# KadAMRN/Data_Free_Quantization

Hardware: AMD Instinct MI355X
Metric: weight-GB/s quantized (per-ch INT8 DFQ sweep) + top-1 delta, MobileNetV2 (higher is better)
Workload: dtype f32

## Files before the change

data_free_quantization_amd/csrc/dfq_sweep.hip:

```cpp
#include "dfq_common.h"
#include "dfq_sweep_plan.h"
#ifdef DFQ_DIAGNOSTICS
#include "dfq_diag.h"
#endif

#include <algorithm>
#include <cstring>
#include <cstdlib>
#include <new>
#include <type_traits>
#include <vector>

namespace dfq {

constexpr int kBlockThreads = kWave * kWavesPerBlock;

__device__ __forceinline__ int64_t task_elem_start(const DevTask& k, const DevTensor& T) { return k.src - T.src; }

template <int CHUNK, int MAXROWS, int NB>
struct LdsLayout {
    static constexpr int kPerWave = NB * CHUNK + 3 * MAXROWS;
    static constexpr int kTotal = kWavesPerBlock * kPerWave;
};

__device__ __forceinline__ bool is_sym(int mode) { return mode == DFQ_TENSOR_SYM || mode == DFQ_CHANNEL_SYM; }

template <bool NT, typename V>
__device__ __forceinline__ void st(V* p, const V& v);

__device__ __forceinline__ void store_code(void* codes, int cb, int64_t idx, float q) {
    if (cb == 1) {
        st<false>(static_cast<int8_t*>(codes) + idx, (int8_t)(int)q);
    } else {
        st<false>(static_cast<int16_t*>(codes) + idx, (int16_t)(int)q);
    }
}

typedef __attribute__((address_space(3))) void lds_void_t;
typedef __attribute__((address_space(1))) void gbl_void_t;

template <bool NT = false>
__device__ __forceinline__ void glds16(const float* g, float* lds_base) {
    __builtin_amdgcn_global_load_lds((gbl_void_t*)g, (lds_void_t*)lds_base, 16, 0, NT ? 2 : 0);
}
template <bool NT = false>
__device__ __forceinline__ void glds4(const float* g, float* lds_base) {
    __builtin_amdgcn_global_load_lds((gbl_void_t*)g, (lds_void_t*)lds_base, 4, 0, NT ? 2 : 0);
}
template <bool NT = false>
__device__ __forceinline__ void glds16_asm(const float* g, float* lds_base) {
    const uint32_t m0 = (uint32_t)(uintptr_t)(lds_void_t*)lds_base;
    if constexpr (NT) asm volatile("global_load_lds_dwordx4 %0, off nt" ::"v"(g), "{m0}"(m0) : "memory");
    else asm volatile("global_load_lds_dwordx4 %0, off" ::"v"(g), "{m0}"(m0) : "memory");
}
template <bool NT = false>
__device__ __forceinline__ void glds4_asm(const float* g, float* lds_base) {
    const uint32_t m0 = (uint32_t)(uintptr_t)(lds_void_t*)lds_base;
    if constexpr (NT) asm volatile("global_load_lds_dword %0, off nt" ::"v"(g), "{m0}"(m0) : "memory");
    else asm volatile("global_load_lds_dword %0, off" ::"v"(g), "{m0}"(m0) : "memory");
}
typedef float f32x4 __attribute__((ext_vector_type(4)));
template <bool NT, typename V>
__device__ __forceinline__ void st(V* p, const V& v) {
    if constexpr (sizeof(V) == 16) {
        const f32x4 w = {v.x, v.y, v.z, v.w};
        DFQ_GLOBAL f32x4* g = (DFQ_GLOBAL f32x4*)p;
        if constexpr (NT) __builtin_nontemporal_store(w, g);
        else *g = w;
    } else {
        DFQ_GLOBAL V* g = (DFQ_GLOBAL V*)p;
        if constexpr (NT) __builtin_nontemporal_store(v, g);
        else *g = v;
    }
}
__device__ __forceinline__ float ld(const float* p) { return *(const DFQ_GLOBAL float*)p; }
__device__ __forceinline__ float4 ld(const float4* p) {
    const f32x4 v = *(const DFQ_GLOBAL f32x4*)p;
    return make_float4(v.x, v.y, v.z, v.w);
}
__device__ __forceinline__ void vm_wait_all() { asm volatile("s_waitcnt vmcnt(0)" ::: "memory"); }

__global__ void __launch_bounds__(kBlockThreads)
sweep_reduce_kernel(const DevTensor* __restrict__ tensors, const DevTask* __restrict__ tasks,
                    int64_t ntasks, uint32_t* __restrict__ slot_min, uint32_t* __restrict__ slot_max) {
    const int lane = threadIdx.x & (kWave - 1);
    const int64_t wave0 = (int64_t)blockIdx.x * kWavesPerBlock + wave_uniform(threadIdx.x >> 6);
    const int64_t nwaves = (int64_t)gridDim.x * kWavesPerBlock;
    for (int64_t t = wave0; t < ntasks; t += nwaves) {
        const DevTask task = tasks[t];
        const float* src = task.src;
        float vmin = INFINITY, vmax = -INFINITY;
        if (task.flags & 2) {
            const int nj = task.n >> 2;
#pragma unroll 8
            for (int j = lane; j < nj; j += kWave) {
                const float4 v = ld(reinterpret_cast<const float4*>(src) + j);
                vmin = fminf(vmin, fminf(fminf(v.x, v.y), fminf(v.z, v.w)));
                vmax = fmaxf(vmax, fmaxf(fmaxf(v.x, v.y), fmaxf(v.z, v.w)));
            }
        } else {
#pragma unroll 8
            for (int e = lane; e < task.n; e += kWave) {
                const float x = ld(src + e);
                vmin = fminf(vmin, x);
                vmax = fmaxf(vmax, x);
            }
        }
        vmin = wave_min(vmin);
        vmax = wave_max(vmax);
        if (lane == 0) {
            atomicMin(&slot_min[task.slot], enc_ord(vmin));
            atomicMax(&slot_max[task.slot], enc_ord(vmax));
        }
    }
}

template <bool NT = false, bool ASM = false>
__device__ __forceinline__ void issue_task_load(const DevTask& task, float* data, int lane) {
    const float* src = task.src;
    const int n = task.n;
    if (task.flags & 2) {
        const int nj = n >> 2;
        for (int m = 0; m * kWave < nj; ++m) {
            const int j = lane + m * kWave;
            if (j < nj) {
                if constexpr (ASM) glds16_asm<NT>(src + 4 * j, data + 4 * kWave * m);
                else glds16<NT>(src + 4 * j, data + 4 * kWave * m);
            }
        }
    } else {
        for (int m = 0; m * kWave < n; ++m) {
            const int e = lane + m * kWave;
            if (e < n) {
                if constexpr (ASM) glds4_asm<NT>(src + e, data + kWave * m);
                else glds4<NT>(src + e, data + kWave * m);
            }
        }
    }
}


typedef float f32x2 __attribute__((ext_vector_type(2)));
template <bool CLIP, int CB, int EM, bool NT>
__device__ __forceinline__ void quant_vec4(const DevTensor& T, int n, int64_t base, float* data, const float* ls,
                                           const float* lmn, const float* lrs, const QParams& pc, bool whole,
                                           int eoff, int lane, float qmin, float qmax, bool sym) {
    constexpr float kMagic = 12582912.0f;
    const int nj = n >> 2;
    float* dq = T.dst + base;
    const float clo = T.clip_lo, chi = T.clip_hi;
    const uint32_t magic = whole ? T.len_magic : 0u;
    const float thr = 0.5f - fmaxf(-qmin, qmax) * 0x1p-20f;
    const f32x2 mg = {kMagic, kMagic};
    struct Q4 {
        float4 x;
        float s, mn;
        float t[4];
        f32x2 ta, tb, qa, qb, da, db;
    };
    auto prep = [&](int j, uint32_t e, Q4& q) {
        q.x = reinterpret_cast<const float4*>(data)[j];
        const uint32_t r = __umulhi(e, magic);
        q.s = ls[r];
        q.mn = lmn[r];
        const float rs = lrs[r];
        const f32x2 nm = {-q.mn, -q.mn};
        const f32x2 rs2 = {rs, rs};
        const f32x2 a = (f32x2{q.x.x, q.x.y} + nm) * rs2, b = (f32x2{q.x.z, q.x.w} + nm) * rs2;
        q.t[0] = __builtin_amdgcn_fmed3f(a.x, qmin, qmax);
        q.t[1] = __builtin_amdgcn_fmed3f(a.y, qmin, qmax);
        q.t[2] = __builtin_amdgcn_fmed3f(b.x, qmin, qmax);
        q.t[3] = __builtin_amdgcn_fmed3f(b.y, qmin, qmax);
        q.ta = f32x2{q.t[0], q.t[1]} + mg;
        q.tb = f32x2{q.t[2], q.t[3]} + mg;
        q.qa = q.ta - mg;
        q.qb = q.tb - mg;
        asm("" : "+v"(q.ta), "+v"(q.tb), "+v"(q.qa), "+v"(q.qb));
        q.da = f32x2{q.t[0], q.t[1]} - q.qa;
        q.db = f32x2{q.t[2], q.t[3]} - q.qb;
    };
    auto dmax = [&](const Q4& q) { return fmaxf(fmaxf(fabsf(q.da.x), fabsf(q.da.y)), fmaxf(fabsf(q.db.x), fabsf(q.db.y))); };
    auto fix = [&](Q4& q) {
        const float negmn = -q.mn;
        if (fabsf(q.da.x) >= thr) q.t[0] = __builtin_amdgcn_fmed3f((q.x.x + negmn) / q.s, qmin, qmax);
        if (fabsf(q.da.y) >= thr) q.t[1] = __builtin_amdgcn_fmed3f((q.x.y + negmn) / q.s, qmin, qmax);
        if (fabsf(q.db.x) >= thr) q.t[2] = __builtin_amdgcn_fmed3f((q.x.z + negmn) / q.s, qmin, qmax);
        if (fabsf(q.db.y) >= thr) q.t[3] = __builtin_amdgcn_fmed3f((q.x.w + negmn) / q.s, qmin, qmax);
        q.ta = f32x2{q.t[0], q.t[1]} + mg;
        q.tb = f32x2{q.t[2], q.t[3]} + mg;
        q.qa = q.ta - mg;
        q.qb = q.tb - mg;
    };
    auto out = [&](int j, const Q4& q) {
        const f32x2 s2 = {q.s, q.s}, mn2 = {q.mn, q.mn};
        const f32x2 ya = q.qa * s2 + mn2, yb = q.qb * s2 + mn2;
        float y[4] = {ya.x, ya.y, yb.x, yb.y};
        if constexpr (CLIP) {
#pragma unroll
            for (int k = 0; k < 4; ++k) y[k] = __builtin_amdgcn_fmed3f(y[k], clo, chi);
        }
        st<NT>(reinterpret_cast<float4*>(dq) + j, make_float4(y[0], y[1], y[2], y[3]));
        const uint32_t u0 = __float_as_uint(q.ta.x), u1 = __float_as_uint(q.ta.y);
        const uint32_t u2 = __float_as_uint(q.tb.x), u3 = __float_as_uint(q.tb.y);
        if constexpr (CB == 1) {
            const uint32_t c = __builtin_amdgcn_perm(u1, u0, 0x0c0c0400u) | __builtin_amdgcn_perm(u3, u2, 0x04000c0cu);
            st<NT>(reinterpret_cast<uint32_t*>(static_cast<uint8_t*>(T.codes) + base) + j, c);
        } else if constexpr (CB == 3) {
            const uint32_t c = (u0 & 0xFu) | ((u1 & 0xFu) << 4) | ((u2 & 0xFu) << 8) | ((u3 & 0xFu) << 12);
            st<NT>(reinterpret_cast<uint16_t*>(static_cast<uint8_t*>(T.codes) + base / 2) + j, (uint16_t)c);
        } else if constexpr (CB == 2) {
            const uint64_t c = (uint64_t)__builtin_amdgcn_perm(u1, u0, 0x05040100u) |
                               ((uint64_t)__builtin_amdgcn_perm(u3, u2, 0x05040100u) << 32);
            st<NT>(reinterpret_cast<uint64_t*>(static_cast<uint16_t*>(T.codes) + base) + j, c);
        }
        if constexpr (EM != 0) {
            const f32x2 ea = f32x2{y[0], y[1]} - f32x2{q.x.x, q.x.y}, eb = f32x2{y[2], y[3]} - f32x2{q.x.z, q.x.w};
            const float4 ev = make_float4(ea.x, ea.y, eb.x, eb.y);
            if constexpr (EM == 1) st<NT>(reinterpret_cast<float4*>(T.esum + base) + j, ev);
            else reinterpret_cast<float4*>(data)[j] = ev;
        }
    };
    uint32_t e = (uint32_t)(4 * lane + eoff);
    for (int j = lane; j < nj; j += 2 * kWave, e += 8 * kWave) {
        const int j1 = j + kWave;
        const bool has1 = j1 < nj;
        Q4 qa, qb;
        prep(j, e, qa);
        prep(has1 ? j1 : j, has1 ? e + 4 * kWave : e, qb);
        if (__builtin_amdgcn_ballot_w64(fmaxf(dmax(qa), dmax(qb)) >= thr)) {
            fix(qa);
            fix(qb);
        }
        out(j, qa);
        if (has1) out(j1, qb);
    }
}

template <bool CLIP, int CB, bool NT>
__device__ __forceinline__ void quant_vec4_e(int em, const DevTensor& T, int n, int64_t base, float* data,
                                             const float* ls, const float* lmn, const float* lrs, const QParams& pc,
                                             bool whole, int eoff, int lane, float qmin, float qmax, bool sym) {
    if (em == 0) quant_vec4<CLIP, CB, 0, NT>(T, n, base, data, ls, lmn, lrs, pc, whole, eoff, lane, qmin, qmax, sym);
    else if (em == 1) quant_vec4<CLIP, CB, 1, NT>(T, n, base, data, ls, lmn, lrs, pc, whole, eoff, lane, qmin, qmax, sym);
    else quant_vec4<CLIP, CB, 2, NT>(T, n, base, data, ls, lmn, lrs, pc, whole, eoff, lane, qmin, qmax, sym);
}

template <bool CLIP, bool NT>
__device__ __forceinline__ void quant_vec4_c(int cb, int em, const DevTensor& T, int n, int64_t base, float* data,
                                             const float* ls, const float* lmn, const float* lrs, const QParams& pc,
                                             bool whole, int eoff, int lane, float qmin, float qmax, bool sym) {
    switch (cb) {
        case 0: quant_vec4_e<CLIP, 0, NT>(em, T, n, base, data, ls, lmn, lrs, pc, whole, eoff, lane, qmin, qmax, sym); break;
        case 1: quant_vec4_e<CLIP, 1, NT>(em, T, n, base, data, ls, lmn, lrs, pc, whole, eoff, lane, qmin, qmax, sym); break;
        case 2: quant_vec4_e<CLIP, 2, NT>(em, T, n, base, data, ls, lmn, lrs, pc, whole, eoff, lane, qmin, qmax, sym); break;
        default: quant_vec4_e<CLIP, 3, NT>(em, T, n, base, data, ls, lmn, lrs, pc, whole, eoff, lane, qmin, qmax, sym);
    }
}

template <int MAXROWS, bool VEC, bool NT = false, int ESPEC = 2, bool SCREEN = true, bool FAST = true>
__device__ __forceinline__ void compute_task(const DevTensor& T, const DevTask& task, float* data, float* ls,
                                             float* lmn, const uint32_t* __restrict__ slot_min,
                                             const uint32_t* __restrict__ slot_max, int lane, float bmn = 0.f,
                                             float bmx = 0.f, int goff = -1, uint64_t* tlm = nullptr,
                                             uint32_t abl = 0) {
    const int n = task.n;
    const bool sym = is_sym(T.mode);
// ... 488 lines not shown
                        gmn = fminf(gmn, b0[q * P + MAXROWS + rr]);
                    }
                }
                block_lds_sync();
                if (rr <= rl) {
                    const QParams p = make_qparams(gmn, gmx, T.bits, is_sym(T.mode), T.flags, T.given_min,
                                                   T.given_max);
                    ls[lane] = p.s;
                    lmn[lane] = p.mn;
                    lmn[MAXROWS + lane] = __builtin_amdgcn_rcpf(p.s);
                    if (rr * len >= g0) {
                        const int64_t row_g = task.row0 + rr;
                        if (T.scale) st<false>(T.scale + row_g, p.s);
                        if (T.zero) st<false>(T.zero + row_g, p.mn);
                    }
                }
                wave_lds_sync();
                goff = g0 - rf * len;
            } else if (task.nrows < 0) {
                float vmin = INFINITY, vmax = -INFINITY;
                if (T.vec4) {
                    for (int j = lane; j < (task.n >> 2); j += kWave) {
                        const float4 v = reinterpret_cast<const float4*>(wl)[j];
                        vmin = fminf(vmin, fminf(fminf(v.x, v.y), fminf(v.z, v.w)));
                        vmax = fmaxf(vmax, fmaxf(fmaxf(v.x, v.y), fmaxf(v.z, v.w)));
                    }
                } else {
                    for (int e = lane; e < task.n; e += kWave) {
                        vmin = fminf(vmin, wl[e]);
                        vmax = fmaxf(vmax, wl[e]);
                    }
                }
                vmin = wave_min(vmin);
                vmax = wave_max(vmax);
                if (lane == 0) {
                    ls[0] = vmin;
                    ls[1] = vmax;
                }
                block_lds_sync();
                constexpr int P = Lay::kPerWave;
                if (task.nrows == -kWavesPerBlock) {
                    const float* b0 = lds + NB * CHUNK;
                    bmn = fminf(fminf(b0[0], b0[P]), fminf(b0[2 * P], b0[3 * P]));
                    bmx = fmaxf(fmaxf(b0[1], b0[P + 1]), fmaxf(b0[2 * P + 1], b0[3 * P + 1]));
                } else {
                    const float* b0 = lds + (w & ~1) * P + NB * CHUNK;
                    bmn = fminf(b0[0], b0[P]);
                    bmx = fmaxf(b0[1], b0[P + 1]);
                }
                block_lds_sync();
            }
            uint64_t marks[4] = {0, 0, 0, 0};
            uint64_t* tlm = TL ? marks : nullptr;
            if (T.vec4)
                compute_task<MAXROWS, true, NT, ESPEC, SCREEN, FAST>(T, task, wl, ls, lmn, slot_min, slot_max, lane,
                                                                     bmn, bmx, goff, tlm, abl);
            else
                compute_task<MAXROWS, false, NT, ESPEC, SCREEN, FAST>(T, task, wl, ls, lmn, slot_min, slot_max, lane,
                                                                      bmn, bmx, goff, tlm, abl);
            if constexpr (TL) {
                if (lane == 0 && t < g_timeline_cap) {
                    uint32_t hw;
                    asm volatile("s_getreg_b32 %0, hwreg(HW_REG_HW_ID)" : "=s"(hw));
                    uint32_t xcc;
                    asm volatile("s_getreg_b32 %0, hwreg(HW_REG_XCC_ID)" : "=s"(xcc));
                    const uint64_t tl2 = wall_clock64();
                    uint64_t* r = g_timeline + 8 * t;
                    r[0] = tl0;
                    r[1] = tl1;
                    r[2] = marks[0];
                    r[3] = marks[1];
                    r[4] = tl2;
                    r[5] = ((uint64_t)task.tensor << 40) | ((uint64_t)(xcc & 0xFF) << 32) | hw;
                    r[6] = marks[2];
                    r[7] = marks[3];
                }
            }
            task = next;
        }
    } else {
        int cur = 0;
        int64_t t = wave0;
        if (t < ntasks) {
            const DevTask task = tasks[t];
            issue_task_load<NT>(task, wl, lane);
        }
        for (; t < ntasks; t += nwaves) {
            const DevTask task = tasks[t];
            const DevTensor T = tensors[task.tensor];
            vm_wait_all();
            wave_lds_sync();
            const int64_t tn = t + nwaves;
            if (tn < ntasks) {
                const DevTask nt = tasks[tn];
                issue_task_load<NT>(nt, wl + (cur ^ 1) * CHUNK, lane);
            }
            float* data = wl + cur * CHUNK;
            if (T.vec4) compute_task<MAXROWS, true, NT, ESPEC, SCREEN>(T, task, data, ls, lmn, slot_min, slot_max, lane);
            else compute_task<MAXROWS, false, NT, ESPEC, SCREEN>(T, task, data, ls, lmn, slot_min, slot_max, lane);
            cur ^= 1;
        }
    }
}

static int lds_bytes(const Variant& V) {
    return 4 * kWavesPerBlock * ((V.prefetch ? 2 : 1) * V.chunk + 3 * V.max_rows);
}

using MainKernel = void (*)(const DevTensor*, const DevTask*, int64_t, const uint32_t*, const uint32_t*);

static MainKernel main_kernel(int variant) {
#define DFQ_V(i) kVariants[i].chunk, kVariants[i].max_rows, kVariants[i].prefetch
#ifndef DFQ_DIAGNOSTICS
    if (variant == kSmallVariant) return sweep_main_kernel<DFQ_V(kSmallVariant), true, 1>;
    return sweep_main_kernel<DFQ_V(kDefaultVariant), true, 1, false, true, true, kDefaultVariant == 16>;
#else
    switch (variant) {
        case 1: return sweep_main_kernel<DFQ_V(1)>;
        case 2: return sweep_main_kernel<DFQ_V(2)>;
        case 3: return sweep_main_kernel<DFQ_V(3)>;
        case 4: return sweep_main_kernel<DFQ_V(4)>;
        case 5: return sweep_main_kernel<DFQ_V(5), true>;
        case 6: return sweep_main_kernel<DFQ_V(6), true, 1>;
        case 7: return sweep_main_kernel<DFQ_V(7), true, 0>;
        case 8: return sweep_main_kernel<DFQ_V(8), true, 1>;
        case 9: return sweep_main_kernel<DFQ_V(9), true, 1>;
        case 10: return sweep_main_kernel<DFQ_V(10), true, 1>;
        case 11: return sweep_main_kernel<DFQ_V(11), true, 1>;
        case 12: return sweep_main_kernel<DFQ_V(12), true, 0>;
        case 13: return sweep_main_kernel<DFQ_V(13), true, 1, true>;
        case 14: return sweep_main_kernel<DFQ_V(14), true, 1, false, false>;
        case 15: return sweep_main_kernel<DFQ_V(15), true, 1, false, true, false>;
        case 16: return sweep_main_kernel<DFQ_V(16), true, 1, false, true, true, true>;
        default: return sweep_main_kernel<DFQ_V(0)>;
    }
#endif
#undef DFQ_V
}

constexpr int kBlocksPerCu = 64;
static int blocks_per_cu() {
    static const int v = [] {
        const char* e = ab_env("DFQ_SWEEP_BLOCKS_PER_CU");
        return e && *e ? std::max(1, std::min(1024, atoi(e))) : kBlocksPerCu;
    }();
    return v;
}
static int grid_for(int64_t ntasks) {
    const int64_t want = ceil_div(ntasks, kWavesPerBlock);
    return (int)std::max<int64_t>(1, std::min<int64_t>(want, 256 * (int64_t)blocks_per_cu()));
}

static int launch_sweep(int variant, hipStream_t s, const DevTensor* t, const DevTask* reduce, int64_t n_reduce,
                        const DevTask* main, int64_t n_main, uint32_t* slots, int64_t n_slots) {
    if (n_reduce > 0) {
        DFQ_HIP_CHECK(hipMemsetAsync(slots, 0xFF, sizeof(uint32_t) * n_slots, s));
        DFQ_HIP_CHECK(hipMemsetAsync(slots + n_slots, 0x00, sizeof(uint32_t) * n_slots, s));
        hipLaunchKernelGGL(sweep_reduce_kernel, dim3(grid_for(n_reduce)), dim3(kBlockThreads), 0, s, t, reduce,
                           n_reduce, slots, slots + n_slots);
        DFQ_LAUNCH_CHECK();
    }
    if (n_main > 0) {
        hipLaunchKernelGGL(main_kernel(variant), dim3(grid_for(n_main)), dim3(kBlockThreads), 0, s, t, main, n_main,
                           slots, slots + n_slots);
        DFQ_LAUNCH_CHECK();
    }
    return DFQ_OK;
}

static std::vector<char> table_blob(const SweepTables& T, size_t o_tensors, size_t o_reduce, size_t o_main,
                                    size_t end) {
    std::vector<char> blob(end - o_tensors, 0);
    auto put = [&](size_t off, const void* p, size_t bytes) {
        if (bytes) std::memcpy(blob.data() + (off - o_tensors), p, bytes);
    };
    put(o_tensors, T.tensors.data(), sizeof(DevTensor) * T.tensors.size());
    put(o_reduce, T.reduce.data(), sizeof(DevTask) * T.reduce.size());
    put(o_main, T.main.data(), sizeof(DevTask) * T.main.size());
    return blob;
}

}

using namespace dfq;

struct dfq_sweep_plan {
    int variant = kDefaultVariant;
    DevTensor* d_tensors = nullptr;
    DevTask* d_reduce = nullptr;
    DevTask* d_main = nullptr;
    uint32_t* d_slots = nullptr;
    void* d_owned = nullptr;
    int64_t n_reduce = 0, n_main = 0, n_slots = 0, n_tensors = 0, n_elems = 0, algo_bytes = 0;
};

static int sweep_plan_create_impl(const dfq_tensor_desc* descs, int32_t n, void* ws, int64_t ws_bytes,
                                  hipStream_t stream, dfq_sweep_plan** out) {
    if (!out || (n > 0 && !descs) || n < 0) return DFQ_ERR_INVALID;
    *out = nullptr;
    SweepTables B;
    PlanLayout Lo;
    int rc = sweep_plan_tables(descs, n, B, Lo);
    if (rc) return rc;
    if (ws && (ws_bytes < Lo.total || reinterpret_cast<uintptr_t>(ws) % 256 != 0)) return DFQ_ERR_WORKSPACE;
    dfq_sweep_plan* p = new (std::nothrow) dfq_sweep_plan();
    if (!p) return DFQ_ERR_NOMEM;
    p->variant = B.variant;
    p->n_reduce = (int64_t)B.reduce.size();
    p->n_main = (int64_t)B.main.size();
    p->n_slots = B.slots;
    p->n_tensors = n;
    p->n_elems = B.elems;
    p->algo_bytes = B.algo_bytes;
    hipError_t e = hipSuccess;
    char* base = static_cast<char*>(ws);
    if (!base) {
        e = hipMalloc(&p->d_owned, Lo.total);
        base = static_cast<char*>(p->d_owned);
    }
    p->d_tensors = reinterpret_cast<DevTensor*>(base + Lo.o_tensors);
    p->d_reduce = reinterpret_cast<DevTask*>(base + Lo.o_reduce);
    p->d_main = reinterpret_cast<DevTask*>(base + Lo.o_main);
    p->d_slots = reinterpret_cast<uint32_t*>(base + Lo.o_slots);
    if (e == hipSuccess) {
        const std::vector<char> blob = table_blob(B, Lo.o_tensors, Lo.o_reduce, Lo.o_main, Lo.o_slots);
        if (ws) {
            e = stage_h2d(base, blob.data(), Lo.o_slots, stream);
        } else {
            e = hipMemcpy(base, blob.data(), Lo.o_slots, hipMemcpyHostToDevice);
        }
    }
    if (e != hipSuccess) {
        set_last_hip_error(e);
        (void)hipFree(p->d_owned);
        delete p;
        return DFQ_ERR_HIP;
    }
    *out = p;
    return DFQ_OK;
}

extern "C" int dfq_sweep_plan_create(const dfq_tensor_desc* descs, int32_t n, dfq_sweep_plan** out) {
    return sweep_plan_create_impl(descs, n, nullptr, 0, nullptr, out);
}

extern "C" int dfq_sweep_plan_create_ws(const dfq_tensor_desc* descs, int32_t n, void* ws, int64_t ws_bytes,
                                        void* stream, dfq_sweep_plan** out) {
    if (!ws) return DFQ_ERR_WORKSPACE;
    return sweep_plan_create_impl(descs, n, ws, ws_bytes, static_cast<hipStream_t>(stream), out);
}

extern "C" int dfq_sweep_plan_execute(dfq_sweep_plan* p, void* stream) {
    if (!p) return DFQ_ERR_INVALID;
    return launch_sweep(p->variant, static_cast<hipStream_t>(stream), p->d_tensors, p->d_reduce, p->n_reduce, p->d_main,
                        p->n_main, p->d_slots, p->n_slots);
}

extern "C" int dfq_sweep_plan_stats(const dfq_sweep_plan* p, dfq_sweep_stats* st) {
    if (!p || !st) return DFQ_ERR_INVALID;
    st->n_tensors = p->n_tensors;
    st->n_elems = p->n_elems;
    st->n_tasks_reduce = p->n_reduce;
    st->n_tasks_main = p->n_main;
    st->algo_bytes = p->algo_bytes;
    st->launches = (p->n_reduce > 0 ? 1 : 0) + (p->n_main > 0 ? 1 : 0);
    st->grid_blocks = p->n_main > 0 ? grid_for(p->n_main) : 0;
    st->variant = p->variant;
    return DFQ_OK;
}

extern "C" int dfq_sweep_plan_destroy(dfq_sweep_plan* p) {
    if (!p) return DFQ_OK;
    (void)hipFree(p->d_owned);
    delete p;
    return DFQ_OK;
}

extern "C" int dfq_quantize_tensor(const dfq_tensor_desc* d, void* ws, size_t ws_bytes, void* stream) {
    if (!d) return DFQ_ERR_INVALID;
    SweepTables B;
    SingleLayout Lo;
    int rc = sweep_single_tables(*d, B, Lo);
    if (rc) return rc;
    if (!ws || ws_bytes < Lo.total) return DFQ_ERR_WORKSPACE;
    hipStream_t s = static_cast<hipStream_t>(stream);
    char* base = static_cast<char*>(ws);
    DevTensor* dt = reinterpret_cast<DevTensor*>(base + Lo.o_tensor);
    const std::vector<char> blob = table_blob(B, Lo.o_tensor, Lo.o_reduce, Lo.o_main, Lo.total);
    DFQ_HIP_CHECK(stage_h2d(dt, blob.data(), blob.size(), s));
    return launch_sweep(B.variant, s, dt, reinterpret_cast<DevTask*>(base + Lo.o_reduce), (int64_t)B.reduce.size(),
                        reinterpret_cast<DevTask*>(base + Lo.o_main), (int64_t)B.main.size(),
                        reinterpret_cast<uint32_t*>(base), B.slots);
}

#ifdef DFQ_DIAGNOSTICS
extern "C" int dfq_debug_timeline(void* buf, int64_t cap) {
    uint64_t* p = static_cast<uint64_t*>(buf);
    DFQ_HIP_CHECK(hipMemcpyToSymbol(HIP_SYMBOL(g_timeline), &p, sizeof(p)));
    DFQ_HIP_CHECK(hipMemcpyToSymbol(HIP_SYMBOL(g_timeline_cap), &cap, sizeof(cap)));
    return DFQ_OK;
}

extern "C" int dfq_debug_ablate(uint32_t flags) {
    DFQ_HIP_CHECK(hipMemcpyToSymbol(HIP_SYMBOL(g_ablate), &flags, sizeof(flags)));
    return DFQ_OK;
}
#endif

namespace dfq {
hipError_t preload_sweep() {
    hipFuncAttributes a;
    hipError_t e = hipFuncGetAttributes(&a, reinterpret_cast<const void*>(main_kernel(kDefaultVariant)));
    if (e == hipSuccess) e = hipFuncGetAttributes(&a, reinterpret_cast<const void*>(sweep_reduce_kernel));
    return e;
}
}
```

data_free_quantization_amd/csrc/dfq_transform.hip:

```cpp
#include "dfq_common.h"
#include "dfq_transform_plan.h"

#include <cstring>

#include <algorithm>
#include <vector>

namespace dfq {

__device__ __forceinline__ float bn_factor(float g, float v, float eps) {
    return g / sqrtf(v + eps);
}

__global__ void bn_fold_weight_kernel(float* __restrict__ w, const float* __restrict__ g,
                                      const float* __restrict__ v, float eps, int64_t rows, int64_t len) {
    const int64_t n = rows * len;
    for (int64_t i = (int64_t)blockIdx.x * blockDim.x + threadIdx.x; i < n; i += (int64_t)gridDim.x * blockDim.x) {
        const int64_t o = i / len;
        w[i] = w[i] * bn_factor(g[o], v[o], eps);
    }
}

__device__ __forceinline__ void bn_fold_channel(const BnFoldJob& J, int64_t o) {
    typedef DFQ_GLOBAL float* G;
    const G g = (G)J.g, b = (G)J.b, m = (G)J.m, v = (G)J.v, bias = (G)J.bias, fw = (G)J.fake_w, fb = (G)J.fake_b;
    const float go = g[o], bo = b[o], mo = m[o], vo = v[o];
    const float f = bn_factor(go, vo, J.eps);
    const float shift = bo - (go * mo) / sqrtf(vo + J.eps);
    const float b0 = (J.flags & DFQ_BN_FOLD_ZERO_BIAS) ? 0.0f : bias[o];
    bias[o] = b0 * f + shift;
    if (J.fake_w) fw[o] = fabsf(go);
    if (J.fake_b) fb[o] = bo;
    g[o] = 1.0f;
    v[o] = 1.0f;
    b[o] = 0.0f;
    m[o] = 0.0f;
}

__global__ void bn_fold_channel_kernel(float* __restrict__ bias, float* __restrict__ g, float* __restrict__ b,
                                       float* __restrict__ m, float* __restrict__ v, float* __restrict__ fake_w,
                                       float* __restrict__ fake_b, float eps, int64_t rows) {
    const BnFoldJob J{nullptr, bias, g, b, m, v, fake_w, fake_b, eps, 0, rows, 0, nullptr};
    for (int64_t o = (int64_t)blockIdx.x * blockDim.x + threadIdx.x; o < rows; o += (int64_t)gridDim.x * blockDim.x)
        bn_fold_channel(J, o);
}

__device__ __forceinline__ float fold_factor(const BnFoldJob& J, int64_t o) {
    const float go = ((const DFQ_GLOBAL float*)J.g)[o], ve = ((const DFQ_GLOBAL float*)J.v)[o] + J.eps;
    return (go == 1.0f && ve == 1.0f) ? 1.0f : go / sqrtf(ve);
}

__device__ __forceinline__ float fold_one(const BnFoldJob& J, int64_t r0, int64_t base, float inv, int64_t i,
                                          float w) {
    int rem;
    const float f = fold_factor(J, fold_row(J.row_len, r0, base, inv, i, &rem));
    return f != 1.0f ? w * f : w;
}

__global__ void __launch_bounds__(kThreads)
bn_fold_weight_batch_kernel(const BnFoldJob* __restrict__ jobs, const BnFoldChunk* __restrict__ chunks,
                            int64_t nchunks) {
    __shared__ float smn[kThreads / kWave], smx[kThreads / kWave];
    for (int64_t c = blockIdx.x; c < nchunks; c += gridDim.x) {
        const BnFoldChunk ch = chunks[c];
        const BnFoldJob J = jobs[ch.job];
        const int64_t r0 = ch.e0 / J.row_len, base = r0 * J.row_len;
        const float inv = 1.0f / (float)J.row_len;
        float a = INFINITY, b = -INFINITY;
        const int64_t n = ch.e1 - ch.e0;
        int64_t done = 0;
        int ident = 1;
        for (int64_t r = r0 + threadIdx.x; r <= (ch.e1 - 1) / J.row_len; r += blockDim.x)
            ident &= fold_factor(J, r) == 1.0f;
        ident = __syncthreads_and(ident);
        if (ident && (reinterpret_cast<uintptr_t>(J.w + ch.e0) & 15) == 0) {
            const DFQ_GLOBAL f32x4* w4 = (const DFQ_GLOBAL f32x4*)(J.w + ch.e0);
            const int64_t n4 = n >> 2;
            for (int64_t k = threadIdx.x; k < n4; k += 4 * (int64_t)blockDim.x) {
                f32x4 v[4];
#pragma unroll
                for (int u = 0; u < 4; ++u)
                    if (k + u * (int64_t)blockDim.x < n4) v[u] = w4[k + u * blockDim.x];
#pragma unroll
                for (int u = 0; u < 4; ++u)
                    if (k + u * (int64_t)blockDim.x < n4) {
                        a = fminf(a, fminf(fminf(v[u].x, v[u].y), fminf(v[u].z, v[u].w)));
                        b = fmaxf(b, fmaxf(fmaxf(v[u].x, v[u].y), fmaxf(v[u].z, v[u].w)));
                    }
            }
            done = 4 * n4;
        } else if ((reinterpret_cast<uintptr_t>(J.w + ch.e0) & 15) == 0) {
            DFQ_GLOBAL f32x4* w4 = (DFQ_GLOBAL f32x4*)(J.w + ch.e0);
            const int64_t n4 = n >> 2;
            for (int64_t k = threadIdx.x; k < n4; k += blockDim.x) {
                const f32x4 v = w4[k];
                const int64_t i = ch.e0 + 4 * k;
                f32x4 o;
                int rem;
                const float f = fold_factor(J, fold_row(J.row_len, r0, base, inv, i, &rem));
                if (rem + 3 < (int)J.row_len) {
                    o.x = f != 1.0f ? v.x * f : v.x;
                    o.y = f != 1.0f ? v.y * f : v.y;
                    o.z = f != 1.0f ? v.z * f : v.z;
                    o.w = f != 1.0f ? v.w * f : v.w;
                } else {
                    o.x = f != 1.0f ? v.x * f : v.x;
                    o.y = fold_one(J, r0, base, inv, i + 1, v.y);
                    o.z = fold_one(J, r0, base, inv, i + 2, v.z);
                    o.w = fold_one(J, r0, base, inv, i + 3, v.w);
                }
                if (__float_as_uint(o.x) != __float_as_uint(v.x) || __float_as_uint(o.y) != __float_as_uint(v.y) ||
                    __float_as_uint(o.z) != __float_as_uint(v.z) || __float_as_uint(o.w) != __float_as_uint(v.w))
                    w4[k] = o;
                a = fminf(a, fminf(fminf(o.x, o.y), fminf(o.z, o.w)));
                b = fmaxf(b, fmaxf(fmaxf(o.x, o.y), fmaxf(o.z, o.w)));
            }
            done = 4 * n4;
        }
        DFQ_GLOBAL float* wg = (DFQ_GLOBAL float*)J.w;
        for (int64_t k = done + threadIdx.x; k < n; k += blockDim.x) {
            const int64_t i = ch.e0 + k;
            const float v = wg[i];
            const float o = fold_one(J, r0, base, inv, i, v);
            if (__float_as_uint(o) != __float_as_uint(v)) wg[i] = o;
            a = fminf(a, o);
            b = fmaxf(b, o);
        }
        if (J.range_enc) {
            block_minmax(a, b, smn, smx);
            if (threadIdx.x == 0) {
                atomicMax(&J.range_enc[0], ~enc_ord(a));
                atomicMax(&J.range_enc[1], enc_ord(b));
            }
            __syncthreads();
        }
    }
}

__global__ void bn_fold_channel_batch_kernel(const BnFoldJob* __restrict__ jobs, int32_t njobs) {
    for (int32_t j = blockIdx.x; j < njobs; j += gridDim.x) {
        const BnFoldJob J = jobs[j];
        for (int64_t o = threadIdx.x; o < J.rows; o += blockDim.x) bn_fold_channel(J, o);
    }
}

constexpr int kClampBatch = 64;
struct ClampBatch {
    float* w[kClampBatch];
    int64_t n[kClampBatch];
};

__global__ void __launch_bounds__(kThreads) clamp_batch_kernel(ClampBatch b, float lo, float hi) {
    float* __restrict__ w = b.w[blockIdx.y];
    const int64_t n = b.n[blockIdx.y];
    const int64_t n4 = n >> 2;
    float4* w4 = reinterpret_cast<float4*>(w);
    for (int64_t i = (int64_t)blockIdx.x * blockDim.x + threadIdx.x; i < n4; i += (int64_t)gridDim.x * blockDim.x) {
        float4 v = w4[i];
        v.x = fminf(fmaxf(v.x, lo), hi);
        v.y = fminf(fmaxf(v.y, lo), hi);
        v.z = fminf(fmaxf(v.z, lo), hi);
        v.w = fminf(fmaxf(v.w, lo), hi);
        w4[i] = v;
    }
    for (int64_t i = 4 * n4 + (int64_t)blockIdx.x * blockDim.x + threadIdx.x; i < n; i += (int64_t)gridDim.x * blockDim.x)
        w[i] = fminf(fmaxf(w[i], lo), hi);
}

__device__ __forceinline__ float absorb_c(float beta, float gamma, float n_sigma) {
    float c = beta - n_sigma * gamma;
    return (c < 0.0f) ? 0.0f : c;
}

__device__ __forceinline__ float absorb_row(const float* w2, const float* bn_w, const float* bn_b, int64_t o,
                                            int64_t i2, int64_t khw2, int64_t o2g, float n_sigma, int lane) {
    const int64_t g = o / o2g;
    const float* row = w2 + o * i2 * khw2;
    float acc = 0.f;
    for (int64_t i = lane; i < i2; i += 64) {
        float ssum = 0.f;
        for (int64_t k = 0; k < khw2; ++k) ssum += row[i * khw2 + k];
        const int64_t ch = g * i2 + i;
        acc += ssum * absorb_c(bn_b[ch], bn_w[ch], n_sigma);
    }
    return wave_sum_f(acc);
}

__global__ void absorb_gemv_kernel(const float* __restrict__ w2, float* __restrict__ b2,
                                   const float* __restrict__ bn_w, const float* __restrict__ bn_b,
                                   int64_t o2, int64_t i2, int64_t khw2, int64_t o2g, float n_sigma) {
    const int lane = threadIdx.x & 63;
    const int64_t wave = (int64_t)blockIdx.x * (blockDim.x / 64) + (threadIdx.x >> 6);
    const int64_t nwaves = (int64_t)gridDim.x * (blockDim.x / 64);
    for (int64_t o = wave; o < o2; o += nwaves) {
        const float acc = absorb_row(w2, bn_w, bn_b, o, i2, khw2, o2g, n_sigma, lane);
        if (lane == 0) b2[o] = b2[o] + acc;
    }
}

__global__ void absorb_channel_kernel(float* __restrict__ b1, float* __restrict__ bn_b, const float* __restrict__ bn_w,
                                      int64_t c1, float n_sigma) {
    for (int64_t c = (int64_t)blockIdx.x * blockDim.x + threadIdx.x; c < c1; c += (int64_t)gridDim.x * blockDim.x) {
        const float cc = absorb_c(bn_b[c], bn_w[c], n_sigma);
        b1[c] = b1[c] + (-cc);
        bn_b[c] = bn_b[c] + (-cc);
    }
}

__global__ void absorb_batch_gemv_kernel(const AbsRel* __restrict__ rels, const AbsRows* __restrict__ tasks,
                                         int64_t ntasks, float* __restrict__ wc, float n_sigma) {
    const int lane = threadIdx.x & 63;
    const int64_t wave = (int64_t)blockIdx.x * (blockDim.x / 64) + (threadIdx.x >> 6);
    const int64_t nwaves = (int64_t)gridDim.x * (blockDim.x / 64);
    for (int64_t t = wave; t < ntasks; t += nwaves) {
        const AbsRows tk = tasks[t];
        const AbsRel R = rels[tk.r];
        for (int64_t o = tk.o0; o < tk.o1; ++o) {
            const float acc = absorb_row(R.w2, R.bn_w, R.bn_b, o, R.i2, R.khw2, R.o2g, n_sigma, lane);
            if (lane == 0) wc[R.wc + o] = acc;
        }
    }
}

__global__ void absorb_batch_bias_kernel(const AbsRel* __restrict__ rels, const AbsVec* __restrict__ vecs,
                                         const AbsOp* __restrict__ ops, const AbsElems* __restrict__ tasks,
                                         int64_t ntasks, const float* __restrict__ wc, float n_sigma) {
    for (int64_t t = blockIdx.x; t < ntasks; t += gridDim.x) {
        const AbsElems tk = tasks[t];
        const AbsVec V = vecs[tk.v];
        for (int64_t e = tk.e0 + threadIdx.x; e < tk.e1; e += blockDim.x) {
            float b = V.b[e];
            for (int32_t q = 0; q < V.nops; ++q) {
                const AbsOp op = ops[V.op0 + q];
                const AbsRel& R = rels[op.r];
                if (op.kind == 0) {
                    b = b + wc[R.wc + e];
                } else {
                    const float cc = absorb_c(R.bn_b[e], R.bn_w[e], n_sigma);
                    b = b + (-cc);
                    R.bn_b[e] = R.bn_b[e] + (-cc);
                }
            }
            V.b[e] = b;
        }
    }
}

}

using namespace dfq;

extern "C" int dfq_bn_fold(float* w, float* bias, float* bn_w, float* bn_b, float* bn_mean, float* bn_var,
                           float* fake_w, float* fake_b, float eps, int64_t rows, int64_t row_len, void* stream) {
    if (!w || !bias || !bn_w || !bn_b || !bn_mean || !bn_var || rows < 0 || row_len < 0) return DFQ_ERR_INVALID;
    if (rows == 0) return DFQ_OK;
    hipStream_t s = static_cast<hipStream_t>(stream);
    hipLaunchKernelGGL(bn_fold_weight_kernel, dim3(blocks_for(rows * row_len, 4)), dim3(kThreads), 0, s,
                       w, bn_w, bn_var, eps, rows, row_len);
    DFQ_LAUNCH_CHECK();
    hipLaunchKernelGGL(bn_fold_channel_kernel, dim3(blocks_for(rows)), dim3(kThreads), 0, s,
                       bias, bn_w, bn_b, bn_mean, bn_var, fake_w, fake_b, eps, rows);
    DFQ_LAUNCH_CHECK();
    return DFQ_OK;
}

extern "C" int dfq_bn_fold_batch(const dfq_bn_fold_desc* d, int32_t n, void* ws, int64_t ws_bytes, void* stream) {
    if (n < 0 || (n > 0 && !d)) return DFQ_ERR_INVALID;
    if (n == 0) return DFQ_OK;
    std::vector<BnFoldJob> jobs;
    std::vector<BnFoldChunk> chunks;
    const int rc = bn_fold_tables(d, n, jobs, chunks);
    if (rc != DFQ_OK) return rc;
    const BnFoldLayout L = bn_fold_layout(d, n);
    const int64_t jb = L.o_chunks, need = L.total;
    if (ws && (ws_bytes < need || reinterpret_cast<uintptr_t>(ws) % 256 != 0)) return DFQ_ERR_INVALID;
    hipStream_t s = static_cast<hipStream_t>(stream);
    void* own = nullptr;
    if (!ws) {
        DFQ_HIP_CHECK(hipMalloc(&own, need));
        ws = own;
    }
    char* base = static_cast<char*>(ws);
    BnFoldJob* dj = reinterpret_cast<BnFoldJob*>(base);
    BnFoldChunk* dc = reinterpret_cast<BnFoldChunk*>(base + jb);
    std::vector<char> blob(need, 0);
    std::memcpy(blob.data(), jobs.data(), sizeof(BnFoldJob) * n);
    if (!chunks.empty()) std::memcpy(blob.data() + jb, chunks.data(), sizeof(BnFoldChunk) * chunks.size());
    hipError_t e = own ? hipMemcpyAsync(base, blob.data(), need, hipMemcpyHostToDevice, s)
                       : stage_h2d(base, blob.data(), need, s);
    std::vector<uint32_t*> rp;
    for (int32_t j = 0; j < n; ++j)
        if (d[j].range_enc) rp.push_back(d[j].range_enc);
    std::sort(rp.begin(), rp.end());
    for (size_t k = 0; k < rp.size() && e == hipSuccess;) {
        size_t m = k + 1;
        while (m < rp.size() && rp[m] == rp[m - 1] + 2) ++m;
        e = hipMemsetAsync(rp[k], 0, sizeof(uint32_t) * 2 * (m - k), s);
        k = m;
    }
    if (e == hipSuccess && !chunks.empty()) {
        hipLaunchKernelGGL(bn_fold_weight_batch_kernel, dim3((int)std::min<size_t>(chunks.size(), 4096)),
                           dim3(kThreads), 0, s, dj, dc, (int64_t)chunks.size());
        e = hipGetLastError();
    }
    if (e == hipSuccess) {
        hipLaunchKernelGGL(bn_fold_channel_batch_kernel, dim3(std::min(n, 2048)), dim3(kThreads), 0, s, dj, n);
        e = hipGetLastError();
    }
    if (e == hipSuccess && own) e = hipStreamSynchronize(s);
    if (own) (void)hipFree(own);
    if (e != hipSuccess) {
        set_last_hip_error(e);
        return DFQ_ERR_HIP;
    }
    return DFQ_OK;
}

extern "C" int dfq_clamp_batch(float* const* w, const int64_t* n, int32_t count, float lo, float hi, void* stream) {
    if (count < 0 || (count > 0 && (!w || !n))) return DFQ_ERR_INVALID;
    for (int32_t k = 0; k < count; ++k)
        if (!w[k] || n[k] < 0 || reinterpret_cast<uintptr_t>(w[k]) % 16) return DFQ_ERR_INVALID;
    for (int32_t k0 = 0; k0 < count; k0 += kClampBatch) {
        ClampBatch b{};
        int cnt = 0;
        int64_t most = 0;
        for (int32_t k = k0; k < std::min(count, k0 + kClampBatch); ++k) {
            if (n[k] == 0) continue;
            b.w[cnt] = w[k];
            b.n[cnt] = n[k];
            most = std::max(most, n[k]);
            ++cnt;
        }
        if (cnt == 0) continue;
        hipLaunchKernelGGL(clamp_batch_kernel, dim3(blocks_for(most, 16), cnt), dim3(kThreads), 0,
                           static_cast<hipStream_t>(stream), b, lo, hi);
        DFQ_LAUNCH_CHECK();
    }
    return DFQ_OK;
}

extern "C" int dfq_clamp(float* w, int64_t n, float lo, float hi, void* stream) {
    return dfq_clamp_batch(&w, &n, 1, lo, hi, stream);
}

extern "C" int dfq_bias_absorb(const float* w2, float* b1, float* b2, float* bn_w, float* bn_b, int64_t c1,
                               int64_t o2, int64_t i2, int64_t khw2, float n_sigma, void* stream) {
    if (!w2 || !b1 || !b2 || !bn_w || !bn_b || c1 <= 0 || o2 <= 0 || i2 <= 0 || khw2 <= 0) return DFQ_ERR_INVALID;
    const int64_t groups = c1 / i2;
    if (groups <= 0 || o2 % groups != 0) return DFQ_ERR_SHAPE;
    const int64_t o2g = o2 / groups;
    if (c1 / groups != i2) return DFQ_ERR_SHAPE;
    hipStream_t s = static_cast<hipStream_t>(stream);
    const int wave_blocks = (int)std::min<int64_t>(ceil_div(o2, kThreads / 64), 2048);
    hipLaunchKernelGGL(absorb_gemv_kernel, dim3(wave_blocks), dim3(kThreads), 0, s, w2, b2, bn_w, bn_b, o2, i2, khw2,
                       o2g, n_sigma);
    DFQ_LAUNCH_CHECK();
    hipLaunchKernelGGL(absorb_channel_kernel, dim3(blocks_for(c1)), dim3(kThreads), 0, s, b1, bn_b, bn_w, c1, n_sigma);
    DFQ_LAUNCH_CHECK();
    return DFQ_OK;
}

extern "C" int dfq_bias_absorb_batch(const dfq_absorb_desc* d, int32_t n, float n_sigma, void* ws, int64_t ws_bytes,
                                     int32_t* failed, void* stream) {
    if (failed) *failed = -1;
    if (n < 0 || (n > 0 && !d)) return DFQ_ERR_INVALID;
    if (n == 0) return DFQ_OK;
    AbsTables T;
    const int rc = absorb_tables(d, n, T, failed);
    if (rc != DFQ_OK) return rc;
    const AbsLayout L = absorb_layout(T);
    if (!ws || ws_bytes < L.total || reinterpret_cast<uintptr_t>(ws) % 256 != 0) return DFQ_ERR_WORKSPACE;
    hipStream_t s = static_cast<hipStream_t>(stream);
    char* base = static_cast<char*>(ws);
    std::vector<char> blob(L.host, 0);
    auto put = [&](int64_t off, const auto& v) {
        if (!v.empty()) std::memcpy(blob.data() + off, v.data(), sizeof(v[0]) * v.size());
    };
    put(L.o_rels, T.rels); put(L.o_rows, T.rows); put(L.o_vecs, T.vecs); put(L.o_ops, T.ops); put(L.o_elems, T.elems);
    DFQ_HIP_CHECK(stage_h2d(base, blob.data(), L.host, s));
    const AbsRel* dr = reinterpret_cast<const AbsRel*>(base + L.o_rels);
    float* wc = reinterpret_cast<float*>(base + L.o_wc);
    const int64_t nrow = (int64_t)T.rows.size(), nel = (int64_t)T.elems.size();
    hipLaunchKernelGGL(absorb_batch_gemv_kernel, dim3((int)std::min<int64_t>(ceil_div(nrow, kThreads / 64), 4096)),
                       dim3(kThreads), 0, s, dr, reinterpret_cast<const AbsRows*>(base + L.o_rows), nrow, wc, n_sigma);
    DFQ_LAUNCH_CHECK();
    hipLaunchKernelGGL(absorb_batch_bias_kernel, dim3((int)std::min<int64_t>(nel, 4096)), dim3(kThreads), 0, s, dr,
                       reinterpret_cast<const AbsVec*>(base + L.o_vecs), reinterpret_cast<const AbsOp*>(base + L.o_ops),
                       reinterpret_cast<const AbsElems*>(base + L.o_elems), nel, wc, n_sigma);
    DFQ_LAUNCH_CHECK();
    return DFQ_OK;
}

namespace dfq {
hipError_t preload_transform() {
    hipFuncAttributes a;
    hipError_t e = hipFuncGetAttributes(&a, reinterpret_cast<const void*>(bn_fold_weight_batch_kernel));
    if (e == hipSuccess) e = hipFuncGetAttributes(&a, reinterpret_cast<const void*>(absorb_batch_gemv_kernel));
    return e;
}
}
```

Measured before the change: 1660.

## Double-buffer min/max range loads with cross-task prefetch and nontemporal hints

Adds a shared range-streaming helper that keeps two register batches of eight float4 loads in flight. While one batch is reduced into min/max, the next is issued, including the first batch of the next task. Both the sweep reduce kernel and the BN-fold identity path now use it. Early tasks get nontemporal loads, while roughly the last 256MB of data is read normally so it can stay in cache for the following pass. The BN-fold grid cap is also raised. The costs are higher register pressure and more complex control flow. Clamped out-of-range loads re-read the last element rather than being skipped.

```diff
diff --git a/data_free_quantization_amd/csrc/dfq_range_stream.h b/data_free_quantization_amd/csrc/dfq_range_stream.h
--- /dev/null
+++ b/data_free_quantization_amd/csrc/dfq_range_stream.h
@@ -0,0 +1,72 @@
+#pragma once
+#include "dfq_common.h"
+
+namespace dfq {
+
+constexpr int kRangeDepth = 8;
+constexpr int64_t kRangeKeepBytes = int64_t(256) << 20;
+struct RangeBatch {
+    f32x4 v[kRangeDepth];
+};
+
+template <typename BytesOf>
+inline int64_t range_nt_count(int64_t count, BytesOf bytes_of) {
+    int64_t kept = 0, i = count;
+    while (i > 0 && kept < kRangeKeepBytes) kept += bytes_of(--i);
+    return i;
+}
+
+template <bool NT>
+__device__ __forceinline__ void range_issue(RangeBatch& B, const DFQ_GLOBAL f32x4* p, int n4, int first, int stride) {
+    const DFQ_GLOBAL char* base = (const DFQ_GLOBAL char*)p;
+    if constexpr (NT) asm volatile("");
+#pragma unroll
+    for (int u = 0; u < kRangeDepth; ++u) {
+        const DFQ_GLOBAL f32x4* q = (const DFQ_GLOBAL f32x4*)(base + 16u * (uint32_t)min(first + u * stride, n4 - 1));
+        if constexpr (NT) B.v[u] = __builtin_nontemporal_load(q);
+        else B.v[u] = *q;
+    }
+    if constexpr (NT) asm volatile("");
+}
+__device__ __forceinline__ void range_issue(RangeBatch& B, const DFQ_GLOBAL f32x4* p, int n4, int first, int stride,
+                                            bool nt) {
+    if (nt) range_issue<true>(B, p, n4, first, stride);
+    else range_issue<false>(B, p, n4, first, stride);
+}
+
+__device__ __forceinline__ void range_take(const RangeBatch& B, float& lo, float& hi) {
+#pragma unroll
+    for (int u = 0; u < kRangeDepth; ++u) {
+        lo = min3_nc(min3_nc(lo, B.v[u].x, B.v[u].y), B.v[u].z, B.v[u].w);
+        hi = max3_nc(max3_nc(hi, B.v[u].x, B.v[u].y), B.v[u].z, B.v[u].w);
+    }
+}
+
+template <bool NT>
+__device__ __forceinline__ bool range_stream(RangeBatch& A, RangeBatch& B, const DFQ_GLOBAL f32x4* p, int n4, int tid,
+                                             int stride, float& lo, float& hi, const DFQ_GLOBAL f32x4* pn, int n4n) {
+    const int step = kRangeDepth * stride;
+    for (int b = step;; b += 2 * step) {
+        const bool last_a = b >= n4;
+        range_issue<NT>(B, last_a ? pn : p, last_a ? n4n : n4, last_a ? tid : b + tid, stride);
+        __builtin_amdgcn_sched_barrier(0);
+        range_take(A, lo, hi);
+        __builtin_amdgcn_sched_barrier(0);
+        if (last_a) return false;
+        const bool last_b = b + step >= n4;
+        range_issue<NT>(A, last_b ? pn : p, last_b ? n4n : n4, last_b ? tid : b + step + tid, stride);
+        __builtin_amdgcn_sched_barrier(0);
+        range_take(B, lo, hi);
+        __builtin_amdgcn_sched_barrier(0);
+        if (last_b) return true;
+    }
+}
+__device__ __forceinline__ bool range_stream(RangeBatch& A, RangeBatch& B, const DFQ_GLOBAL f32x4* p, int n4, int tid,
+                                             int stride, bool nt, float& lo, float& hi, const DFQ_GLOBAL f32x4* pn,
+                                             int n4n) {
+    return nt ? range_stream<true>(A, B, p, n4, tid, stride, lo, hi, pn, n4n)
+              : range_stream<false>(A, B, p, n4, tid, stride, lo, hi, pn, n4n);
+}
+__device__ __forceinline__ const DFQ_GLOBAL f32x4* range_none(const DFQ_GLOBAL f32x4* p, int n4) { return p + (n4 - 1); }
+
+}
diff --git a/data_free_quantization_amd/csrc/dfq_sweep.hip b/data_free_quantization_amd/csrc/dfq_sweep.hip
--- a/data_free_quantization_amd/csrc/dfq_sweep.hip
+++ b/data_free_quantization_amd/csrc/dfq_sweep.hip
@@ -1,4 +1,5 @@
 #include "dfq_common.h"
+#include "dfq_range_stream.h"
 #include "dfq_sweep_plan.h"
 #ifdef DFQ_DIAGNOSTICS
 #include "dfq_diag.h"
@@ -82,36 +83,52 @@
 
 __global__ void __launch_bounds__(kBlockThreads)
 sweep_reduce_kernel(const DevTensor* __restrict__ tensors, const DevTask* __restrict__ tasks,
-                    int64_t ntasks, uint32_t* __restrict__ slot_min, uint32_t* __restrict__ slot_max) {
+                    int64_t ntasks, int64_t nt_tasks, uint32_t* __restrict__ slot_min, uint32_t* __restrict__ slot_max) {
     const int lane = threadIdx.x & (kWave - 1);
     const int64_t wave0 = (int64_t)blockIdx.x * kWavesPerBlock + wave_uniform(threadIdx.x >> 6);
     const int64_t nwaves = (int64_t)gridDim.x * kWavesPerBlock;
-    for (int64_t t = wave0; t < ntasks; t += nwaves) {
-        const DevTask task = tasks[t];
-        const float* src = task.src;
+    if (wave0 >= ntasks) return;
+    int64_t t = wave0;
+    DevTask task = tasks[t];
+    typedef const DFQ_GLOBAL f32x4* Src;
+    auto vecs = [](const DevTask& k) { return (k.flags & 2) ? k.n >> 2 : 0; };
+    auto step = [&](RangeBatch& cur, RangeBatch& oth) __attribute__((always_inline)) -> int {
+        const bool more = t + nwaves < ntasks;
+        DevTask next = task;
+        if (more) next = tasks[t + nwaves];
+        const bool ahead = more && vecs(next) > 0;
         float vmin = INFINITY, vmax = -INFINITY;
-        if (task.flags & 2) {
-            const int nj = task.n >> 2;
+        bool in_cur = false;
+        if (vecs(task) > 0) {
+            const Src p = (Src)task.src;
+            in_cur = range_stream(cur, oth, p, vecs(task), lane, kWave, t < nt_tasks, vmin, vmax,
+                                  ahead ? (Src)next.src : range_none(p, vecs(task)), ahead ? vecs(next) : 1);
+        } else {
+            if (ahead) range_issue(oth, (Src)next.src, vecs(next), lane, kWave, t + nwaves < nt_tasks);
+            if (!(task.flags & 2)) {
 #pragma unroll 8
-            for (int j = lane; j < nj; j += kWave) {
-                const float4 v = ld(reinterpret_cast<const float4*>(src) + j);
-                vmin = fminf(vmin, fminf(fminf(v.x, v.y), fminf(v.z, v.w)));
-                vmax = fmaxf(vmax, fmaxf(fmaxf(v.x, v.y), fmaxf(v.z, v.w)));
-            }
-        } else {
-#pragma unroll 8
-            for (int e = lane; e < task.n; e += kWave) {
-                const float x = ld(src + e);
-                vmin = fminf(vmin, x);
-                vmax = fmaxf(vmax, x);
-            }
-        }
-        vmin = wave_min(vmin);
-        vmax = wave_max(vmax);
+                for (int e = lane; e < task.n; e += kWave) {
+                    const float x = ld(task.src + e);
+                    vmin = fminf(vmin, x);
+                    vmax = fmaxf(vmax, x);
+                }
+            }
+        }
+        group_minmax(vmin, vmax, kWave);
         if (lane == 0) {
             atomicMin(&slot_min[task.slot], enc_ord(vmin));
             atomicMax(&slot_max[task.slot], enc_ord(vmax));
         }
+        task = next;
+        t += nwaves;
+        return !more ? 0 : (in_cur ? 2 : 1);
+    };
+    RangeBatch A, B;
+    if (vecs(task) > 0) range_issue(A, (Src)task.src, vecs(task), lane, kWave, t < nt_tasks);
+    for (bool in_b = false;;) {
+        const int r = in_b ? step(B, A) : step(A, B);
+        if (r == 0) break;
+        in_b ^= r == 1;
     }
 }
 
@@ -906,12 +923,12 @@
 }
 
 static int launch_sweep(int variant, hipStream_t s, const DevTensor* t, const DevTask* reduce, int64_t n_reduce,
-                        const DevTask* main, int64_t n_main, uint32_t* slots, int64_t n_slots) {
+                        int64_t nt_reduce, const DevTask* main, int64_t n_main, uint32_t* slots, int64_t n_slots) {
     if (n_reduce > 0) {
         DFQ_HIP_CHECK(hipMemsetAsync(slots, 0xFF, sizeof(uint32_t) * n_slots, s));
         DFQ_HIP_CHECK(hipMemsetAsync(slots + n_slots, 0x00, sizeof(uint32_t) * n_slots, s));
         hipLaunchKernelGGL(sweep_reduce_kernel, dim3(grid_for(n_reduce)), dim3(kBlockThreads), 0, s, t, reduce,
-                           n_reduce, slots, slots + n_slots);
+                           n_reduce, nt_reduce, slots, slots + n_slots);
         DFQ_LAUNCH_CHECK();
     }
     if (n_main > 0) {
@@ -920,6 +937,10 @@
         DFQ_LAUNCH_CHECK();
     }
     return DFQ_OK;
+}
+
+static int64_t reduce_nt_tasks(const SweepTables& T) {
+    return range_nt_count((int64_t)T.reduce.size(), [&](int64_t k) { return (int64_t)4 * T.reduce[k].n; });
 }
 
 static std::vector<char> table_blob(const SweepTables& T, size_t o_tensors, size_t o_reduce, size_t o_main,
@@ -946,6 +967,7 @@
     uint32_t* d_slots = nullptr;
     void* d_owned = nullptr;
     int64_t n_reduce = 0, n_main = 0, n_slots = 0, n_tensors = 0, n_elems = 0, algo_bytes = 0;
+    int64_t nt_reduce = 0;
 };
 
 static int sweep_plan_create_impl(const dfq_tensor_desc* descs, int32_t n, void* ws, int64_t ws_bytes,
@@ -961,6 +983,7 @@
     if (!p) return DFQ_ERR_NOMEM;
     p->variant = B.variant;
     p->n_reduce = (int64_t)B.reduce.size();
+    p->nt_reduce = reduce_nt_tasks(B);
     p->n_main = (int64_t)B.main.size();
     p->n_slots = B.slots;
     p->n_tensors = n;
@@ -1006,8 +1029,8 @@
 
 extern "C" int dfq_sweep_plan_execute(dfq_sweep_plan* p, void* stream) {
     if (!p) return DFQ_ERR_INVALID;
-    return launch_sweep(p->variant, static_cast<hipStream_t>(stream), p->d_tensors, p->d_reduce, p->n_reduce, p->d_main,
-                        p->n_main, p->d_slots, p->n_slots);
+    return launch_sweep(p->variant, static_cast<hipStream_t>(stream), p->d_tensors, p->d_reduce, p->n_reduce,
+                        p->nt_reduce, p->d_main, p->n_main, p->d_slots, p->n_slots);
 }
 
 extern "C" int dfq_sweep_plan_stats(const dfq_sweep_plan* p, dfq_sweep_stats* st) {
@@ -1043,7 +1066,7 @@
     const std::vector<char> blob = table_blob(B, Lo.o_tensor, Lo.o_reduce, Lo.o_main, Lo.total);
     DFQ_HIP_CHECK(stage_h2d(dt, blob.data(), blob.size(), s));
     return launch_sweep(B.variant, s, dt, reinterpret_cast<DevTask*>(base + Lo.o_reduce), (int64_t)B.reduce.size(),
-                        reinterpret_cast<DevTask*>(base + Lo.o_main), (int64_t)B.main.size(),
+                        reduce_nt_tasks(B), reinterpret_cast<DevTask*>(base + Lo.o_main), (int64_t)B.main.size(),
                         reinterpret_cast<uint32_t*>(base), B.slots);
 }
 
diff --git a/data_free_quantization_amd/csrc/dfq_transform.hip b/data_free_quantization_amd/csrc/dfq_transform.hip
--- a/data_free_quantization_amd/csrc/dfq_transform.hip
+++ b/data_free_quantization_amd/csrc/dfq_transform.hip
@@ -1,4 +1,5 @@
 #include "dfq_common.h"
+#include "dfq_range_stream.h"
 #include "dfq_transform_plan.h"
 
 #include <cstring>
@@ -59,7 +60,7 @@
 
 __global__ void __launch_bounds__(kThreads)
 bn_fold_weight_batch_kernel(const BnFoldJob* __restrict__ jobs, const BnFoldChunk* __restrict__ chunks,
-                            int64_t nchunks) {
+                            int64_t nchunks, int64_t nt_chunks) {
     __shared__ float smn[kThreads / kWave], smx[kThreads / kWave];
     for (int64_t c = blockIdx.x; c < nchunks; c += gridDim.x) {
         const BnFoldChunk ch = chunks[c];
@@ -69,26 +70,20 @@
         float a = INFINITY, b = -INFINITY;
         const int64_t n = ch.e1 - ch.e0;
         int64_t done = 0;
+        const bool vec = (reinterpret_cast<uintptr_t>(J.w + ch.e0) & 15) == 0 && n >= 4;
+        const DFQ_GLOBAL f32x4* s4 = (const DFQ_GLOBAL f32x4*)(J.w + ch.e0);
+        const bool nt = c < nt_chunks;
+        RangeBatch first;
+        if (vec) range_issue(first, s4, (int)(n >> 2), (int)threadIdx.x, (int)blockDim.x, nt);
         int ident = 1;
         for (int64_t r = r0 + threadIdx.x; r <= (ch.e1 - 1) / J.row_len; r += blockDim.x)
             ident &= fold_factor(J, r) == 1.0f;
         ident = __syncthreads_and(ident);
-        if (ident && (reinterpret_cast<uintptr_t>(J.w + ch.e0) & 15) == 0) {
-            const DFQ_GLOBAL f32x4* w4 = (const DFQ_GLOBAL f32x4*)(J.w + ch.e0);
-            const int64_t n4 = n >> 2;
-            for (int64_t k = threadIdx.x; k < n4; k += 4 * (int64_t)blockDim.x) {
-                f32x4 v[4];
-#pragma unroll
-                for (int u = 0; u < 4; ++u)
-                    if (k + u * (int64_t)blockDim.x < n4) v[u] = w4[k + u * blockDim.x];
-#pragma unroll
-                for (int u = 0; u < 4; ++u)
-                    if (k + u * (int64_t)blockDim.x < n4) {
-                        a = fminf(a, fminf(fminf(v[u].x, v[u].y), fminf(v[u].z, v[u].w)));
-                        b = fmaxf(b, fmaxf(fmaxf(v[u].x, v[u].y), fmaxf(v[u].z, v[u].w)));
-                    }
-            }
-            done = 4 * n4;
+        if (ident && vec) {
+            RangeBatch second;
+            range_stream(first, second, s4, (int)(n >> 2), (int)threadIdx.x, (int)blockDim.x, nt, a, b,
+                         range_none(s4, (int)(n >> 2)), 1);
+            done = n & ~(int64_t)3;
         } else if ((reinterpret_cast<uintptr_t>(J.w + ch.e0) & 15) == 0) {
             DFQ_GLOBAL f32x4* w4 = (DFQ_GLOBAL f32x4*)(J.w + ch.e0);
             const int64_t n4 = n >> 2;
@@ -299,8 +294,10 @@
         k = m;
     }
     if (e == hipSuccess && !chunks.empty()) {
-        hipLaunchKernelGGL(bn_fold_weight_batch_kernel, dim3((int)std::min<size_t>(chunks.size(), 4096)),
-                           dim3(kThreads), 0, s, dj, dc, (int64_t)chunks.size());
+        const int64_t nt_chunks =
+            range_nt_count((int64_t)chunks.size(), [&](int64_t c) { return 4 * (chunks[c].e1 - chunks[c].e0); });
+        hipLaunchKernelGGL(bn_fold_weight_batch_kernel, dim3((int)std::min<size_t>(chunks.size(), 16384)),
+                           dim3(kThreads), 0, s, dj, dc, (int64_t)chunks.size(), nt_chunks);
         e = hipGetLastError();
     }
     if (e == hipSuccess) {
```

After: 1663, median of 2. No clear change (+0.2%).
